# Tianion/topazdb

Measured on AMD Instinct MI355X. Metric: GiB/s device-resident SSTable block decode+checksum, 4KiB blocks, 1 MI355X, higher is better.
Workload: dtype u8; 1 GPU; 4k: 1048576 blocks/GPU x 4155 B median, 34.0 entries/block, tag 1 (Uncompress); blocks_per_gpu=1048576, input_bytes_per_gpu=4356833280, parallelism=shard1

## Files before the change

### topazdb_amd/csrc/tpz_decode.hip

```cpp

#include <hip/hip_runtime.h>
#include <stdint.h>

#include "tpz_internal.h"
#include "tpz_spill.hip"

namespace tpz {

typedef uint32_t u32;
typedef uint64_t u64;

constexpr int kWave = 64;
#ifdef TPZ_ABL_W20
#ifdef TPZ_ABL_W8
constexpr int kWavesPerWG = 8;
#else
constexpr int kWavesPerWG = 10;
#endif
#else
constexpr int kWavesPerWG = 16;
#endif
constexpr int kWGThreads = kWave * kWavesPerWG;
constexpr u32 kRowShift = 4, kRowBlocks = 1u << kRowShift;
#ifndef TPZ_ROW_AHEAD
// ... 508 lines not shown
      const uint4 v = src((int)x0 + delta);
      acc.x = (acc.x & ~byte_mask(lo, hi, 0)) | (v.x & byte_mask(lo, hi, 0));
      acc.y = (acc.y & ~byte_mask(lo, hi, 1)) | (v.y & byte_mask(lo, hi, 1));
      acc.z = (acc.z & ~byte_mask(lo, hi, 2)) | (v.z & byte_mask(lo, hi, 2));
      acc.w = (acc.w & ~byte_mask(lo, hi, 3)) | (v.w & byte_mask(lo, hi, 3));
    }
  }
  dst.put(c, acc, act);
  return carry_out;
}

template <class Col, class MapT, class S, class D>
__device__ __forceinline__ void copy_stream(const S& src, const Col& col, const MapT* map, u32 nk,
                                            u32 tot, const D& dst, u32 map_len) {
  const u32 lane = lane_id();
  const u32 nch = (tot + 15) >> 4;
  const u32 npad = (nch + 7) & ~7u;
  const u32 nw = (npad + 63) >> 6;
#ifdef TPZ_ABL_MEMONLY
  for (u32 c = lane; c < npad; c += 64) dst.put(c, make_uint4(c, 0, 0, 0), c < nch);
  return;
#endif
  u32 carry = 0;
  for (u32 w = 0; w < nw; w++) carry = copy_window(src, col, map, nk, tot, dst, map_len, w, carry);
}

struct PendingCrc {
  u32 live;
  u32 b, st, cnt, stored, k;
  u32 lc;
  u32 early;
};

__device__ __forceinline__ void finish_pending(const u32* tab, const Out& o, PendingCrc& pd) {
  if (!pd.live) return;
  const u32 R = crc_combine(tab, pd.lc);
  const u32 crc = (R == crc_shift_small(tab, ~pd.stored, pd.k)) ? pd.stored
                                                                   : ~crc_unshift_small(tab, R, pd.k);
  const bool ok = crc == pd.stored;
  put_meta(o, pd.b, ok ? pd.st : TPZ_BLOCK_CHECKSUM_MISMATCH, ok ? pd.cnt : 0u, crc);
  pd.live = 0;
}

struct FinishAtExit {
  const u32* tab;
  const Out& o;
  PendingCrc& pd;
  bool on;
  __device__ __forceinline__ ~FinishAtExit() {
    if (on) finish_pending(tab, o, pd);
  }
};

template <int J>
__device__ __forceinline__ bool comb_lane(u32 lane) {
  return J == 0 ? (lane & 1u) == 1u : J == 1 ? (lane & 3u) == 2u : J == 2 ? (lane & 7u) == 4u
       : J == 3 ? (lane & 15u) == 8u : J == 4 ? (lane & 31u) == 16u : (lane & 47u) == 32u;
}
struct CombLv {
  u32 r0, r1, r2, r3;
};
template <int J>
__device__ __forceinline__ CombLv comb_issue(const u32* tab, u32 A) {
  CombLv c;
  if (comb_lane<J>(lane_id())) {
    constexpr int b0 = 16 + 4 * J;
    c.r0 = tlook(tab, b0, A & 0xFF);
    c.r1 = tlook(tab, b0 + 1, (A >> 8) & 0xFF);
    c.r2 = tlook(tab, b0 + 2, (A >> 16) & 0xFF);
    c.r3 = tlook(tab, b0 + 3, A >> 24);
  }
  return c;
}
template <int J>
__device__ __forceinline__ u32 comb_use(u32 A, const CombLv& c) {
  if (comb_lane<J>(lane_id())) A = xor3(c.r0, c.r1, c.r2) ^ c.r3;
  if (J < 4) A ^= dpp<kRowShl + (1 << (J < 4 ? J : 0))>(A);
  return A;
}

__device__ __forceinline__ void comb_finish(const u32* tab, const Out& o, PendingCrc& pd, u32 cA,
                                            u32 want) {
  if (!pd.live) return;
  const u32 R = readlane(cA, 0) ^ readlane(cA, 16) ^ readlane(cA, 32) ^ readlane(cA, 48);
  const u32 crc = R == want ? pd.stored : ~crc_unshift_small(tab, R, pd.k);
  const bool ok = crc == pd.stored;
  put_meta(o, pd.b, ok ? pd.st : TPZ_BLOCK_CHECKSUM_MISMATCH, ok ? pd.cnt : 0u, crc);
  pd.live = 0;
}

struct CrcLane {
  int seg;
  bool act;
  u32 c;
};

__device__ __forceinline__ void crc_step(const u32* tab, const uint8_t* win, int pb, CrcLane& L,
                                         int t) {
  typedef u32 u32x4 __attribute__((ext_vector_type(4)));
  const int a = L.act ? pb + L.seg + 16 * t : -kGuard;
  const u32x4 w = *reinterpret_cast<const u32x4*>(win + a);
  L.c = slice16(tab, w.x ^ L.c, w.y, w.z, w.w);
}
__device__ __forceinline__ u32 crc_lane_value(const u32* tab, const CrcLane& L) { return L.c; }

struct FastWin {
  u32 nk, tot, nch, npad, last;
  __amdgpu_buffer_rsrc_t out;
};

template <bool FLAT, class S>
__device__ __forceinline__ u32 copy_fast(const S& src, const ColSmall& col, const uint16_t* map,
                                         const FastWin& F, const FlatOut& D, u32 w, u32 carry,
                                         u32& rare) {
  const u32 lane = lane_id();
  const u32 c = 64 * w + lane;
  const u32 x0 = 16 * c;
  const bool act = c < F.nch;
  u32 j = map[min(c, (u32)kWaveMapLen - 1)];
  j = max(wave_scan_max(act ? j : 0u), carry);
  const u32 carry_out = readlane(j, 63);
  u32 e0, e1;
  int d0, d1;
  col.get2(min(j, F.last), e0, d0, e1, d1);
  const bool cross = act && j + 1 < F.nk && e0 < x0 + 16;
  uint4 acc = src(act ? (int)x0 + d0 : -kGuard);
  const uint4 nx = src(cross ? (int)x0 + d1 : -kGuard);
  const bool rw = __ballot(act && (e0 <= x0 || (cross && e1 < x0 + 16 && j + 2 < F.nk))) != 0;
  if (rw) rare |= 1u << w;
  if (cross) acc = merge_at(acc, nx, (int)(e0 - x0));
  if (FLAT) {
    D.put(c, acc, rw);
  } else {
    __builtin_amdgcn_raw_buffer_store_b128(__builtin_bit_cast(__attribute__((ext_vector_type(4))) u32, acc),
                                           F.out, rw ? kOob : x0, 0, 0);
  }
  return carry_out;
}

template <bool FLAT, class S>
__device__ __forceinline__ u32 copy_fast3(const S& src, const ColSmall& col, const uint16_t* map,
                                          const FastWin& F, const FlatOut& D, u32 w, u32 carry,
                                          u32& rare) {
  const u32 lane = lane_id();
  const u32 c = 64 * w + lane;
  const u32 x0 = 16 * c;
  const bool act = c < F.nch;
  u32 j = map[min(c, (u32)kWaveMapLen - 1)];
  j = max(wave_scan_max(act ? j : 0u), carry);
  const u32 carry_out = readlane(j, 63);
  u32 e0, e1, e2, e3;
  int d0, d1, d2, d3;
  col.get2(min(j, F.last), e0, d0, e1, d1);
  col.get2(min(j + 2, F.last), e2, d2, e3, d3);
  if (act && e0 <= x0) {
    j++;
    e0 = e1, d0 = d1, e1 = e2, d1 = d2, e2 = e3, d2 = d3;
  }
  const bool b1 = act && j + 1 < F.nk && e0 < x0 + 16;
  const bool b2 = b1 && j + 2 < F.nk && e1 < x0 + 16;
  uint4 acc = src(act ? (int)x0 + d0 : -kGuard);
  const uint4 n1 = src(b1 ? (int)x0 + d1 : -kGuard);
  const uint4 n2 = src(b2 ? (int)x0 + d2 : -kGuard);
  const bool rw = __ballot(act && (e0 <= x0 || (b2 && e2 < x0 + 16 && j + 3 < F.nk))) != 0;
  if (rw) rare |= 1u << w;
  if (b1) acc = merge_at(acc, n1, (int)(e0 - x0));
  if (b2) acc = merge_at(acc, n2, (int)(e1 - x0));
  if (FLAT)
    D.put(c, acc, rw);
  else
    __builtin_amdgcn_raw_buffer_store_b128(__builtin_bit_cast(__attribute__((ext_vector_type(4))) u32, acc),
                                           F.out, rw ? kOob : x0, 0, 0);
  return carry_out;
}

template <bool SHORT, bool FLAT, class S>
__device__ __forceinline__ u32 copy_crc_fused(const u32* tab, const S& src, const ColSmall& col,
                                              const uint16_t* map, u32 nk, u32 tot, uint8_t* dst,
                                              const FlatOut& D, const uint8_t* win, int pb, u32 Pa,
                                              u32 kshift, Stamps& St, u32 w3, const Out& o,
                                              PendingCrc& pd) {
  const u32 lane = lane_id();
  FastWin F;
  F.nk = nk;
  F.tot = tot;
  F.nch = (tot + 15) >> 4;
  F.npad = FLAT ? F.nch : (F.nch + 7) & ~7u;
  F.last = nk ? nk - 1 : 0u;
  F.out = __builtin_amdgcn_make_buffer_rsrc(dst, (short)0, FLAT ? 0 : (int)(F.npad * 16), 0x00020000);
  const u32 nw = (F.npad + 63) >> 6;
  CrcLane L;
  L.seg = (int)Pa - kCrcLaneBytes * (int)(lane + 1);
  L.act = L.seg + kCrcLaneBytes > 0;
  L.c = 0;
  u32 carry = 0, rare = 0, cw[5];
  const bool pl = pd.live != 0;
  u32 cA = pd.lc, want = 0;
  CombLv cl{0u, 0u, 0u, 0u};
  if (pl) {
    cl = comb_issue<0>(tab, cA);
    want = crc_shift_small(tab, ~pd.stored, pd.k);
  }
#pragma unroll
  for (int t = 0; t < 4; t++) {
    cw[t] = carry;
    crc_step(tab, win, pb, L, t);
    carry = (SHORT && (u32)t < w3) ? copy_fast3<FLAT>(src, col, map, F, D, (u32)t, carry, rare)
                                   : copy_fast<FLAT>(src, col, map, F, D, (u32)t, carry, rare);
    if (pl) {
      if (t == 0) { cA = comb_use<0>(cA, cl); cl = comb_issue<1>(tab, cA); }
      if (t == 1) { cA = comb_use<1>(cA, cl); cl = comb_issue<2>(tab, cA); }
      if (t == 2) { cA = comb_use<2>(cA, cl); cl = comb_issue<3>(tab, cA); }
      if (t == 3) { cA = comb_use<3>(cA, cl); cl = comb_issue<4>(tab, cA); }
    }
  }
  cw[4] = carry;
  crc_step(tab, win, pb, L, 4);
  if (pl) {
    cA = comb_use<4>(cA, cl);
    cl = comb_issue<5>(tab, cA);
  }
  if (nw > 4)
    carry = (SHORT && 4u < w3) ? copy_fast3<FLAT>(src, col, map, F, D, 4u, carry, rare)
                               : copy_fast<FLAT>(src, col, map, F, D, 4u, carry, rare);
  if (pl) comb_finish(tab, o, pd, comb_use<5>(cA, cl), want);
  TPZ_STAMP(St, 4);
#ifdef TPZ_ABL_STAMPS
  St.rare += __builtin_popcount(rare);
#endif
  if (rare) {
    for (u32 w = 0; w < nw; w++)
      if (rare & (1u << w)) {
        if (FLAT)
          copy_window(src, col, map, nk, F.tot, FlatDst{&D}, (u32)kWaveMapLen, w, cw[w]);
        else
          copy_window(src, col, map, nk, F.tot, SlotDst{dst, F.npad, F.tot}, (u32)kWaveMapLen, w, cw[w]);
      }
  }
  return crc_lane_value(tab, L);
}

typedef u32 u32x2v __attribute__((ext_vector_type(2)));
typedef u32 u32x4v __attribute__((ext_vector_type(4)));
struct Gath {
  u32 d0, d1, d2, d3, d4;
};
__device__ __forceinline__ Gath gath_issue(const uint8_t* base, int x) {
  const u32* p = reinterpret_cast<const u32*>(base + (x & ~3));
  Gath g;
  g.d0 = p[0];
  g.d1 = p[1];
  g.d2 = p[2];
  g.d3 = p[3];
  g.d4 = p[4];
  return g;
}
__device__ __forceinline__ uint4 gath_finish(Gath g, int x) {
  asm volatile("" : "+v"(g.d0), "+v"(g.d1), "+v"(g.d2), "+v"(g.d3), "+v"(g.d4));
  const u32 s = (u32)x & 3u;
  return make_uint4(__builtin_amdgcn_alignbyte(g.d1, g.d0, s), __builtin_amdgcn_alignbyte(g.d2, g.d1, s),
                    __builtin_amdgcn_alignbyte(g.d3, g.d2, s), __builtin_amdgcn_alignbyte(g.d4, g.d3, s));
}
struct Look16 {
  u32 r[16];
};
__device__ __forceinline__ Look16 look_issue(const u32* tab, u32x4v w, u32 c) {
  Look16 L;
  const u32 w0 = w.x ^ c;
#pragma unroll
  for (int i = 0; i < 4; i++) {
    L.r[i] = tlook(tab, 15 - i, (w0 >> (8 * i)) & 0xFF);
    L.r[4 + i] = tlook(tab, 11 - i, (w.y >> (8 * i)) & 0xFF);
    L.r[8 + i] = tlook(tab, 7 - i, (w.z >> (8 * i)) & 0xFF);
    L.r[12 + i] = tlook(tab, 3 - i, (w.w >> (8 * i)) & 0xFF);
  }
  return L;
}
__device__ __forceinline__ u32 look_xor(const Look16& L) {
  u32 c = xor3(L.r[0], L.r[1], L.r[2]);
  c = xor3(c, L.r[3], L.r[4]);
  c = xor3(c, L.r[5], L.r[6]);
  c = xor3(c, L.r[7], L.r[8]);
  c = xor3(c, L.r[9], L.r[10]);
  c = xor3(c, L.r[11], L.r[12]);
  c = xor3(c, L.r[13], L.r[14]);
  return c ^ L.r[15];
}
#define TPZ_SB() __builtin_amdgcn_sched_barrier(0)

struct PWin {
  u32 m, j;
  u32 e0, e1;
  int d0, d1;
  bool act, cross;
  Gath ga, gn;
};
struct PWin3 {
  u32 e2, e3;
  int d2, d3;
  bool b2;
  Gath g2;
};

template <bool FLAT, u32 K3>
__device__ __forceinline__ u32 copy_crc_piped(const u32* tab, const ColSmall& col,
                                              const uint16_t* map, u32 nk, u32 tot, uint8_t* dst,
                                              const FlatOut& D, const uint8_t* win, int pb, u32 Pa,
                                              const Out& o, PendingCrc& pd, u32 k3n = K3) {
  const u32 lane = lane_id();
  FastWin F;
  F.nk = nk;
  F.tot = tot;
  F.nch = (tot + 15) >> 4;
  F.npad = FLAT ? F.nch : (F.nch + 7) & ~7u;
  F.last = nk ? nk - 1 : 0u;
  F.out = __builtin_amdgcn_make_buffer_rsrc(dst, (short)0, FLAT ? 0 : (int)(F.npad * 16), 0x00020000);
  const u32 nw = (F.npad + 63) >> 6;
  const int seg = (int)Pa - kCrcLaneBytes * (int)(lane + 1);
  const bool cact = seg + kCrcLaneBytes > 0;
  const int cbase = cact ? pb + seg : -kGuard;
  auto dread = [&](int t) -> u32x4v {
    return *reinterpret_cast<const u32x4v*>(win + cbase + 16 * t);
  };
  PWin W[4];
  PWin3 W3;
#pragma unroll
  for (int w = 0; w < 4; w++) {
    const u32 c = 64 * w + lane;
    W[w].act = c < F.nch;
    W[w].m = map[min(c, (u32)kWaveMapLen - 1)];
  }
  u32x4v dA = dread(0);
  u32 cA = pd.lc;
  CombLv cl = comb_issue<0>(tab, cA);
  const u32 want = crc_shift_small(tab, ~pd.stored, pd.k);
  TPZ_SB();
#pragma unroll
  for (int w = 0; w < 4; w++) W[w].j = wave_scan_max(W[w].act ? W[w].m : 0u);
  u32 cw[5];
  cw[0] = 0;
#pragma unroll
  for (int w = 0; w < 4; w++) {
    W[w].j = max(W[w].j, cw[w]);
    cw[w + 1] = readlane(W[w].j, 63);
  }
#pragma unroll
  for (int w = 0; w < 4; w++) col.get2(min(W[w].j, F.last), W[w].e0, W[w].d0, W[w].e1, W[w].d1);
  if (K3) col.get2(min(W[0].j + 2, F.last), W3.e2, W3.d2, W3.e3, W3.d3);
  cA = comb_use<0>(cA, cl);
  cl = comb_issue<1>(tab, cA);
  TPZ_SB();
  Look16 LK = look_issue(tab, dA, 0u);
  u32x4v dB = dread(1);
  cA = comb_use<1>(cA, cl);
  cl = comb_issue<2>(tab, cA);
  TPZ_SB();
  u32 rare = 0;
  auto gissue = [&](PWin& P, u32 w) {
    const u32 x0 = 16 * (64 * w + lane);
    if (w < K3 && w < k3n) {
      if (w > 0) col.get2(min(P.j + 2, F.last), W3.e2, W3.d2, W3.e3, W3.d3);
      if (P.act && P.e0 <= x0) {
        P.j++;
        P.e0 = P.e1, P.d0 = P.d1, P.e1 = W3.e2, P.d1 = W3.d2, W3.e2 = W3.e3, W3.d2 = W3.d3;
      }
      P.cross = P.act && P.j + 1 < F.nk && P.e0 < x0 + 16;
      W3.b2 = P.cross && P.j + 2 < F.nk && P.e1 < x0 + 16;
      if (__ballot(P.act && (P.e0 <= x0 || (W3.b2 && W3.e2 < x0 + 16 && P.j + 3 < F.nk))) != 0)
        rare |= 1u << w;
      W3.g2 = gath_issue(win, W3.b2 ? (int)x0 + W3.d2 : -kGuard);
    } else {
      P.cross = P.act && P.j + 1 < F.nk && P.e0 < x0 + 16;
    }
    P.ga = gath_issue(win, P.act ? (int)x0 + P.d0 : -kGuard);
    P.gn = gath_issue(win, P.cross ? (int)x0 + P.d1 : -kGuard);
  };
  auto finish = [&](PWin& P, u32 w) {
    const u32 c = 64 * w + lane;
    const u32 x0 = 16 * c;
    const bool rw = w < K3 && w < k3n && (rare & (1u << w));
    uint4 acc = gath_finish(P.ga, P.act ? (int)x0 + P.d0 : -kGuard);
    const uint4 nx = gath_finish(P.gn, P.cross ? (int)x0 + P.d1 : -kGuard);
    if (P.cross) acc = merge_at(acc, nx, (int)(P.e0 - x0));
    if (w < K3 && w < k3n) {
      const uint4 n2 = gath_finish(W3.g2, W3.b2 ? (int)x0 + W3.d2 : -kGuard);
      if (W3.b2) acc = merge_at(acc, n2, (int)(P.e1 - x0));
    }
    if (FLAT)
      D.put(c, acc, rw);
    else
      __builtin_amdgcn_raw_buffer_store_b128(__builtin_bit_cast(u32x4v, acc), F.out, rw ? kOob : x0, 0, 0);
  };
  gissue(W[0], 0);
  cA = comb_use<2>(cA, cl);
  cl = comb_issue<3>(tab, cA);
  TPZ_SB();
  u32 crc = 0;
  crc = look_xor(LK);
  LK = look_issue(tab, dB, crc);
  dA = dread(2);
  cA = comb_use<3>(cA, cl);
  cl = comb_issue<4>(tab, cA);
  TPZ_SB();
  finish(W[0], 0);
  gissue(W[1], 1);
  cA = comb_use<4>(cA, cl);
  cl = comb_issue<5>(tab, cA);
  TPZ_SB();
  crc = look_xor(LK);
  LK = look_issue(tab, dA, crc);
  dB = dread(3);
  cA = comb_use<5>(cA, cl);
  comb_finish(tab, o, pd, cA, want);
  TPZ_SB();
  finish(W[1], 1);
  gissue(W[2], 2);
  TPZ_SB();
  crc = look_xor(LK);
  LK = look_issue(tab, dB, crc);
  dA = dread(4);
  TPZ_SB();
  finish(W[2], 2);
  gissue(W[3], 3);
  TPZ_SB();
  crc = look_xor(LK);
  LK = look_issue(tab, dA, crc);
  TPZ_SB();
  finish(W[3], 3);
  TPZ_SB();
  crc = look_xor(LK);
  if (nw > 4) {
    (void)copy_fast<FLAT>(Src16{win}, col, map, F, D, 4u, cw[4], rare);
  }
  if (rare) {
    for (u32 w = 0; w < nw; w++)
      if (rare & (1u << w)) {
        if (FLAT)
          copy_window(Src16{win}, col, map, nk, F.tot, FlatDst{&D}, (u32)kWaveMapLen, w, cw[w]);
        else
          copy_window(Src16{win}, col, map, nk, F.tot, SlotDst{dst, F.npad, F.tot}, (u32)kWaveMapLen, w, cw[w]);
      }
  }
  return crc;
}


template <class Col, class MapT, int kMapLen, bool BIG, bool FLAT = false>
__device__ __forceinline__ void decode_block(const u32* tab, uint8_t* win, const Col& col,
                                             MapT* map, u32 a0, u32 len, u32 b, u64 ext_b,
                                             const Out& o, u32 kshift, Stamps& S, PendingCrc& pd,
                                             u64 kf = 0, u64 vf = 0, u64 ef = 0,
                                             const Out* o_lds = nullptr) {
  const u32 lane = lane_id();
  const u32 tag = win[(int)(a0 + len) - 1];
  const u32 stored = bswap32(lds_u32(win, len >= 5 ? a0 + len - 5 : a0));
  const u32 n = lds_be16(win, a0);
  const u32 dk = (u32)kf & 15u, dv = (u32)vf & 15u;
  u32 e_off = 0, e_kl = 0;
  bool e_ok = false;
  if (!BIG) {
    e_off = lds_be16(win, a0 + 2 + 2 * lane);
    const u32 Pn = len - 5, db0 = a0 + 2 + 2 * n;
    e_ok = len >= 7 && lane < n && Pn >= 2 + 2 * n && e_off + 2 <= Pn - 2 - 2 * n;
    e_kl = lds_be16(win, e_ok ? db0 + e_off : a0);
  }
  if (pd.early) finish_pending(tab, o, pd);
  FinishAtExit fin{tab, o, pd, true};
  if (len == 0) { put_meta(o, b, TPZ_BLOCK_EMPTY, 0, 0); return; }
  if (tag == 0 || tag > 3) { put_meta(o, b, TPZ_BLOCK_BAD_TAG, 0, 0); return; }
  if (tag != 1) { put_meta(o, b, TPZ_BLOCK_UNSUPPORTED_CODEC, 0, 0); return; }
  if (len - 1 < 4) { put_meta(o, b, TPZ_BLOCK_MALFORMED, 0, 0); return; }
  const u32 P = len - 5;
  const int pb = (int)a0;
  u32 st = TPZ_BLOCK_OK, cnt = n;
  bool fuse = false;
  bool f_short = false;
  u32 f_w3 = 0;
  u32 f_nk = 0, f_tot = 0;
  uint8_t* f_dst = nullptr;
  FlatOut fo;
  if (P < 2 || P < 2 + 2 * n) {
    st = TPZ_BLOCK_MALFORMED;
    cnt = 0;
  } else if (!BIG && n > kWaveMaxN) {
    const Out& oc = o_lds ? *o_lds : o;
    if (FLAT) defer_to(oc.spill_list, oc.spill_count, b);
    else defer_to(oc.defer_list, oc.defer_count, b);
    return;
  } else {
    const u32 db = a0 + 2 + 2 * n;
    const u32 dl = P - 2 - 2 * n;
    const bool slots_fit = FLAT || 6u * n <= len;
    uint2* ends_g = reinterpret_cast<uint2*>(o.ends) + uni64((FLAT || o.efirst) ? ef : entry_base(ext_b, b));
    const u32 n_pad = o.efirst ? n : (n + 15) & ~15u;
    {
      constexpr u32 per = 16 / sizeof(MapT);
      const u32 nz = min((u32)kMapLen, ((len >> 4) + 3 + per - 1) / per * per);
      for (u32 i = lane; i < nz / per; i += 64)
        reinterpret_cast<uint4*>(map)[i] = make_uint4(0, 0, 0, 0);
    }
    u32 ktot = 0, knz_all = 0;
    if (n > 64) {
      for (u32 g0 = 0; g0 < n; g0 += 64) {
        const u32 i = g0 + lane;
        u32 kl = 0;
        if (i < n) {
          const u32 off = lds_be16(win, a0 + 2 + 2 * i);
          if (off + 2 <= dl) {
            kl = lds_be16(win, db + off);
            if (off + 4 + kl > dl) kl = 0;
          }
        }
        knz_all += __builtin_popcountll(__ballot(kl != 0));
        ktot += readlane(wave_scan_incl(kl), 63);
      }
    }
    u32 kc = 0, vc = 0, knz = 0, vnz = 0;
    bool bad = false, short_k = false, short_v = false;
    for (u32 g0 = 0; g0 < n; g0 += 64) {
      const u32 i = g0 + lane;
      const bool act = i < n;
      u32 off = 0, kl = 0, vl = 0;
      bool ok = true;
      if (act) {
        if (!BIG && g0 == 0) {
          off = e_off;
          ok = e_ok;
          if (ok) { kl = e_kl; ok = off + 4 + kl <= dl; }
        } else {
          off = lds_be16(win, a0 + 2 + 2 * i);
          ok = off + 2 <= dl;
          if (ok) { kl = lds_be16(win, db + off); ok = off + 4 + kl <= dl; }
        }
        if (ok) { vl = lds_be16(win, db + off + 2 + kl); ok = off + 4 + kl + vl <= dl; }
        if (!ok) kl = vl = 0;
      }
      bad |= __ballot(act && !ok) != 0;
      short_k |= __ballot(kl != 0 && kl < 16) != 0;
      short_v |= __ballot(vl != 0 && vl < 16) != 0;
      const u32 ki = wave_scan_incl(kl) + kc;
      const u32 vi = wave_scan_incl(vl) + vc;
      const u64 kmask = __ballot(kl != 0), vmask = __ballot(vl != 0);
      if (n <= 64) {
        ktot = readlane(ki, 63);
        knz_all = __builtin_popcountll(kmask);
      }
      const u32 vs = stream_vstart<FLAT>(ktot, dk, dv);
      __builtin_amdgcn_raw_buffer_store_b64(
          __builtin_bit_cast(__attribute__((ext_vector_type(2))) u32,
                             act ? make_uint2(ki, vi) : make_uint2(0, 0)),
          whole_rsrc(ends_g), (slots_fit && i < n_pad) ? 8 * i : kOob, 0, 0);
      if (act && slots_fit) {
        if (kl) {
          const u32 m = knz + lanes_below(kmask);
          const u32 ke = ki + dk;
          col.put(m, ke, (int)(db + off + 2) - (int)(ke - kl));
          if (((ke + 15) >> 4) < (u32)kMapLen) map[(ke + 15) >> 4] = (MapT)(m + 1);
        }
        if (vl) {
          const u32 m = knz_all + vnz + lanes_below(vmask);
          const u32 ve = vs + vi;
          col.put(m, ve, (int)(db + off + 4 + kl) - (int)(ve - vl));
          if (((ve + 15) >> 4) < (u32)kMapLen) map[(ve + 15) >> 4] = (MapT)(m + 1);
        }
      }
      knz += __builtin_popcountll(kmask);
      vnz += __builtin_popcountll(vmask);
      kc = readlane(ki, 63);
      vc = readlane(vi, 63);
    }

    const u32 vs = stream_vstart<FLAT>(kc, dk, dv);
    TPZ_STAMP(S, 2);
    if (bad || !slots_fit || vs + vc > len + (FLAT ? 47u : 2u)) {
      const Out& oc = o_lds ? *o_lds : o;
      defer_to(oc.spill_list, oc.spill_count, b);
      return;
    } else {
      if (BIG) {
        asm volatile("s_waitcnt vmcnt(0)" ::: "memory");
        __builtin_amdgcn_fence(__ATOMIC_RELEASE, "workgroup");
      }
      __builtin_amdgcn_wave_barrier();
      const u32 tot = FLAT ? (vc ? vs + vc : (kc ? dk + kc : 0u)) : vs + vc;
#ifndef TPZ_ABL_NOCOPY
#if !defined(TPZ_ABL_NOCRC) && !defined(TPZ_ABL_MEMONLY)
#ifdef TPZ_ABL_UNFUSED
      if (false) {
#else
      if (!BIG && P >= 4) {
#endif
        fuse = true;
        f_w3 = short_v ? 5u : (short_k ? (((FLAT ? dk : 0u) + kc + 15) / 16 + 63) / 64 : 0u);
        f_short = f_w3 != 0;
        f_nk = knz + vnz;
        f_tot = tot;
        f_dst = FLAT ? nullptr : o.data + slot_base(ext_b, b);
        if (FLAT) fo = flat_out(o, kf, vf, kc, vc);
      } else
#endif
      if (FLAT) {
        fo = flat_out(o, kf, vf, kc, vc);
        copy_stream(Src16{win}, col, map, knz + vnz, tot, FlatDst{&fo}, (u32)kMapLen);
      } else {
        const u32 nch = (tot + 15) >> 4;
        copy_stream(Src16{win}, col, map, knz + vnz, tot,
                    SlotDst{o.data + slot_base(ext_b, b), (nch + 7) & ~7u, tot}, (u32)kMapLen);
      }
#endif
    }
    TPZ_STAMP(S, 3);
  }
  __builtin_amdgcn_wave_barrier();
  u32 crc;
  if (P >= 4) {
    const u32 k = ((a0 + P + 15) & ~15u) - (a0 + P);
    if (lane < 4) win[a0 + lane] ^= 0xFFu;
    if (lane < 16) win[a0 + P + lane] = 0;
    __builtin_amdgcn_wave_barrier();
#if defined(TPZ_ABL_NOCRC) || defined(TPZ_ABL_MEMONLY)
    crc = stored;
#else
    u32 R;
    if (!BIG && fuse) {
      u32 lc;
      fin.on = false;
      if (!f_short) {
        lc = copy_crc_piped<FLAT, 0u>(tab, *reinterpret_cast<const ColSmall*>(&col),
                                         reinterpret_cast<const uint16_t*>(map), f_nk, f_tot, f_dst,
                                         fo, win, pb, P + k, o, pd);
      } else if (f_w3 <= 2u) {
        lc = copy_crc_piped<FLAT, 2u>(tab, *reinterpret_cast<const ColSmall*>(&col),
                                      reinterpret_cast<const uint16_t*>(map), f_nk, f_tot, f_dst,
                                      fo, win, pb, P + k, o, pd, FLAT ? 2u : f_w3);
        f_short = false;
      } else
      {
        lc = f_short
          ? copy_crc_fused<true, FLAT>(tab, Src16{win}, *reinterpret_cast<const ColSmall*>(&col),
                                       reinterpret_cast<const uint16_t*>(map), f_nk, f_tot, f_dst,
                                       fo, win, pb, P + k, kshift, S, f_w3, o, pd)
          : copy_crc_fused<false, FLAT>(tab, Src16{win}, *reinterpret_cast<const ColSmall*>(&col),
                                        reinterpret_cast<const uint16_t*>(map), f_nk, f_tot, f_dst,
                                        fo, win, pb, P + k, kshift, S, 5u, o, pd);
      }
      pd = PendingCrc{1u, b, st, cnt, stored, k, lc, f_short ? 1u : 0u};
      return;
    } else {
        R = wave_crc(tab, win, pb, P + k);
    }
    if constexpr (BIG)
      crc = (R == crc_shift_small(tab, ~stored, k)) ? stored : ~crc_unshift_small(tab, R, k);
    else
      crc = (R == crc_shift_small(tab, ~stored, k)) ? stored : ~crc_unshift_small(tab, R, k);
#endif
  } else {
    u32 c = 0xFFFFFFFFu;
    for (u32 i = 0; i < P; i++) {
      c ^= win[a0 + i];
      for (int k = 0; k < 8; k++) c = (c >> 1) ^ (0xEDB88320u & (0u - (c & 1u)));
    }
    crc = ~c;
  }
  if (crc != stored) {
    st = TPZ_BLOCK_CHECKSUM_MISMATCH;
    cnt = 0;
  }
  TPZ_STAMP(S, 6);
  put_meta(o, b, st, cnt, crc);
}

__device__ __forceinline__ void load_tables(u32* tab, const u32* gtab, int bytes = kTableBytes) {
  const uint4* s = reinterpret_cast<const uint4*>(gtab);
  uint4* d = reinterpret_cast<uint4*>(tab);
  for (int i = threadIdx.x; i < bytes / 16; i += blockDim.x) d[i] = s[i];
  __syncthreads();
}

__device__ __forceinline__ __amdgpu_buffer_rsrc_t window_rsrc(const uint8_t* src, u64 src_bytes,
                                                               u64 wstart) {
  u64 rem = src_bytes > wstart ? src_bytes - wstart : 0;
  if (rem > 0x7FFFFFF0ull) rem = 0x7FFFFFF0ull;
  return __builtin_amdgcn_make_buffer_rsrc((void*)(src + wstart), (short)0, (int)rem, 0x00020000);
}

__device__ __forceinline__ void fix_tail(uint4& v, const uint8_t* src, u64 piece, u64 src_bytes) {
  const bool straddle = piece + 16 > src_bytes && piece < src_bytes;
  if (__ballot(straddle)) {
    u32 w[4] = {0, 0, 0, 0};
#pragma unroll
    for (u32 k = 0; k < 16; k++) {
      const u64 a = piece + k;
      const u32 byte = src[a < src_bytes ? a : src_bytes - 1];
      w[k >> 2] |= (a < src_bytes ? byte : 0u) << (8 * (k & 3));
    }
    v.x = straddle ? w[0] : v.x;
    v.y = straddle ? w[1] : v.y;
    v.z = straddle ? w[2] : v.z;
    v.w = straddle ? w[3] : v.w;
  }
}

struct Params {
  u64* big_scratch;
  u64* spill_used;
  const uint8_t* src;
  const u64* ext;
  u64 src_bytes;
  u32 n_blocks;
  const u32* crc_tables;
  Out out;
  u32 xp[kBigSuper];
  u32 lane_shift[64];
  u32 chunk_shift;
  u32* row_ctr;
  u32* err;
};


template <class T>
__device__ __forceinline__ T const_load(const T* base, u64 i) {
  return reinterpret_cast<const __attribute__((address_space(4))) T*>(reinterpret_cast<uintptr_t>(base))[i];
}

#ifdef TPZ_ABL_ROWLATE
__device__ __noinline__ void rowlate_delay(const Params& p, u32 wid, u32 point) {
  const u32 rows = (p.n_blocks + kRowBlocks - 1) / kRowBlocks;
  const u32 ctr = __hip_atomic_load(p.row_ctr, __ATOMIC_RELAXED, __HIP_MEMORY_SCOPE_AGENT);
  const bool late = point == 0 ? (wid & 1u) != 0 : (wid & 3u) == 2;
  if (late && ctr + 2 * gridDim.x >= rows)
    for (int i = 0; i < 30; i++) __builtin_amdgcn_s_sleep(127);
}
#endif
#ifdef TPZ_ABL_ONCHIP
constexpr u32 kOnchipMask = 4095;
#endif
template <bool FLAT, u32 CS>
#if defined(TPZ_ABL_W20) && !defined(TPZ_ABL_NOCAP)
__global__ __launch_bounds__(kWGThreads) __attribute__((amdgpu_waves_per_eu(5, 5)))
#else
__global__ __launch_bounds__(kWGThreads, 4)
#endif
void decode_wave_kernel(Params p) {
  __shared__ __attribute__((aligned(16))) uint8_t lds[kWaveLds];
  u32* tab = reinterpret_cast<u32*>(lds);
  __shared__ u32 chunk_next;
  __shared__ Out out_lds;
  __shared__ u64 row_ent[kRowRing];
  __shared__ u32 claims_done, exit_slot;
  if (threadIdx.x == 0) {
    claims_done = 0;
    exit_slot = ~0u;
  }
  if (threadIdx.x < kRowAhead && CS < kRowShift) {
    const u32 r0 = atomicAdd(p.row_ctr, 1u);
    row_ent[threadIdx.x] = (u64)r0 | (u64)threadIdx.x << 32;
    if ((u64)r0 * kRowBlocks >= p.n_blocks) {
      claims_done = 1;
      atomicMin(&exit_slot, kRowAhead);
    }
  } else if (threadIdx.x < kRowRing) {
    row_ent[threadIdx.x] = ~0ull;
  }
  if (threadIdx.x == 0) {
    chunk_next = 0;
    out_lds = p.out;
  }
  if (blockIdx.x == 0 && threadIdx.x == 0) *p.spill_used = 0;
  load_tables(tab, p.crc_tables, kWaveTabBytes);

  const u32 wid = uni(threadIdx.x >> 6);
  const u32 lane = lane_id();
  const u32 kshift = p.lane_shift[lane];
  uint8_t* slot = lds + kWaveTabBytes + wid * kSlotBytes;
  uint8_t* win = slot + kGuard;
  uint8_t* etab = win + kWinBytes + 32;
  const ColSmall col{reinterpret_cast<u32*>(etab)};
  uint16_t* map = reinterpret_cast<uint16_t*>(etab + kWaveTabSlots * 4);

  if (lane < kGuard / 16) reinterpret_cast<uint4*>(slot)[lane] = make_uint4(0, 0, 0, 0);
  const u32 nw = gridDim.x * kWavesPerWG;
  Stamps S;
#ifdef TPZ_ABL_STAMPS
  S.last = stamp_now();
#endif

#ifdef TPZ_WAVE_CHUNK
  const u32 cshift = __builtin_ctz((u32)TPZ_WAVE_CHUNK);
#else
  const u32 cshift = CS;
#endif
  const u32 kChunk = 1u << cshift, rshift = kRowShift - cshift;
  u32 pend_slot = ~0u, pend_row = 0;
  const u32 kq = 1u << rshift;
  auto publish = [&]() {
    if (pend_slot != ~0u) {
      if (lane == 0) {

        if ((u64)pend_row * kRowBlocks >= p.n_blocks) {
          __hip_atomic_store(&claims_done, 1u, __ATOMIC_RELAXED, __HIP_MEMORY_SCOPE_WORKGROUP);
          const u32 Q = __hip_atomic_fetch_add(&chunk_next, 0u, __ATOMIC_RELAXED,
                                               __HIP_MEMORY_SCOPE_WORKGROUP);
          atomicMin(&exit_slot, Q == 0 ? kRowAhead : (Q - 1) / kq + kRowAhead + 1);
        }
        __hip_atomic_store(&row_ent[pend_slot % kRowRing], (u64)pend_row | (u64)pend_slot << 32,
                           __ATOMIC_RELAXED, __HIP_MEMORY_SCOPE_WORKGROUP);
      }
      pend_slot = ~0u;
    }
  };
  const bool dyn_rows = rshift != 0;
  u32 q_tk = 0;
  if (lane == 0) q_tk = atomicAdd(&chunk_next, 1u);
  auto claim_chunk = [&]() -> u32 {
    for (;;) {
      publish();
      const u32 q_old = q_tk;
      if (lane == 0) q_tk = atomicAdd(&chunk_next, 1u);
      const u32 q = uni(q_old);
      if (!dyn_rows) {
        const u64 f = ((u64)q * gridDim.x + blockIdx.x) * kRowBlocks;
        return f < p.n_blocks ? (u32)f : p.n_blocks;
      }
      const u32 slot_q = q >> rshift;
      if (slot_q >= uni(__hip_atomic_load(&exit_slot, __ATOMIC_RELAXED, __HIP_MEMORY_SCOPE_WORKGROUP)))
        return p.n_blocks;
      if ((q & ((1u << rshift) - 1u)) == 0) {
#ifdef TPZ_ABL_ROWLATE
        rowlate_delay(p, wid, 0);
#endif
        if (!uni(__hip_atomic_load(&claims_done, __ATOMIC_RELAXED, __HIP_MEMORY_SCOPE_WORKGROUP))) {
          pend_slot = slot_q + kRowAhead;
#ifdef TPZ_ABL_ROWLATE
          rowlate_delay(p, wid, 1);
#endif
          if (lane == 0) pend_row = atomicAdd(p.row_ctr, 1u);
        } else if (lane == 0) {
          const u32 sx = slot_q + kRowAhead;
          __hip_atomic_store(&row_ent[sx % kRowRing], (u64)kRowExit | (u64)sx << 32, __ATOMIC_RELAXED,
                             __HIP_MEMORY_SCOPE_WORKGROUP);
        }
      }
      u32 row = 0;
      if (lane == 0) {
        u32 spins = 0;
        u64 ent;
        while ((u32)((ent = __hip_atomic_load(&row_ent[slot_q % kRowRing], __ATOMIC_RELAXED,
                                              __HIP_MEMORY_SCOPE_WORKGROUP)) >> 32) != slot_q) {
          const u32 rs = (u32)(ent >> 32);
          if (rs != ~0u && (int)(rs - slot_q) > 0) {
            atomicOr(p.err, 4u);
            break;
          }
          __builtin_amdgcn_s_sleep(2);
          if (++spins == (1u << 22)) {
            atomicOr(p.err, 2u);
            break;
          }
        }
        row = (u32)(ent >> 32) != slot_q ? kRowExit : (u32)ent;
      }
      row = uni(row);
      if (row != kRowExit) {
        const u64 f = (u64)row * kRowBlocks + ((q & ((1u << rshift) - 1u)) << cshift);
        if (f < p.n_blocks) return (u32)f;
      }
    }
  };
  auto chunk_first = [](u32 f) -> u32 { return f; };
  u64 gs_cur, gs_nxt;
  auto load_group = [&](u32 q, u64& gs) {
#ifdef TPZ_ABL_ONCHIP
    u32 bb = (chunk_first(q) & kOnchipMask) + (lane <= kChunk ? lane : 0u);
#else
    u32 bb = chunk_first(q) + (lane <= kChunk ? lane : 0u);
#endif
    bb = bb < p.n_blocks ? bb : p.n_blocks;
    gs = p.ext[bb];
  };
  auto lane64 = [](u64 x, u32 l) { return ((u64)readlane((u32)(x >> 32), l) << 32) | readlane((u32)x, l); };
  auto triage_group = [&](u32 q, u64 gs) {
    const u32 glo = (u32)__builtin_amdgcn_update_dpp((int)readlane((u32)gs, 16), (int)(u32)gs,
                                                     kRowShl + 1, 0xF, 0xF, false);
    const u32 ghi = (u32)__builtin_amdgcn_update_dpp((int)readlane((u32)(gs >> 32), 16),
                                                     (int)(u32)(gs >> 32), kRowShl + 1, 0xF, 0xF, false);
    const u64 ge = ((u64)ghi << 32) | glo;
    const u32 cf = chunk_first(q), bb = cf + lane;
    const bool lng = lane < kChunk && lane < p.n_blocks - cf && ge - gs > kWaveMaxLen;
    if (!__ballot(lng)) return;
    const Out& oc = out_lds;
    u32 nent = 0xFFFFu;
    if (lng) nent = ((u32)p.src[gs] << 8) | p.src[gs + 1];
    const bool to_bw = lng && nent < 64 && oc.bw_list && ge - gs <= TPZ_BIGWAVE_BLOCK_BYTES;
    const bool to_spill = lng && !to_bw && (FLAT || ge - gs > kBigMaxLen);
    if (oc.bw_list) defer_lanes(oc.bw_list, oc.bw_count, to_bw, (u32)bb);
    defer_lanes(oc.spill_list, oc.spill_count, to_spill, (u32)bb);
    defer_lanes(oc.defer_list, oc.defer_count, lng && !to_bw && !to_spill, (u32)bb);
  };
  u32 q_cur = claim_chunk(), q_nxt = claim_chunk();
  load_group(q_cur, gs_cur);
  load_group(q_nxt, gs_nxt);
  triage_group(q_cur, gs_cur);
  u32 j = 0;
  u32 b = chunk_first(q_cur);

  uint4 v[kWinRounds];
  u64 s_cur = 0, e_cur = 0;
  u64 kf_cur = 0, vf_cur = 0, ef_cur = 0;
  auto issue = [&](u32 bb, u32 jj, u64& s, u64& e) {
    if (FLAT && bb >= p.n_blocks) return;
    if (bb < p.n_blocks) {
      if (FLAT) {
        kf_cur = const_load(p.out.kfirst, bb);
        vf_cur = const_load(p.out.vfirst, bb);
        ef_cur = const_load(p.out.efirst, bb);
      } else if (p.out.efirst) {
        ef_cur = const_load(p.out.efirst, bb);
      }
    }
    s = lane64(gs_cur, jj);
    e = lane64(gs_cur, jj + 1);
    const bool take = bb < p.n_blocks && e - s <= kWaveMaxLen;
// ... 514 lines not shown
```

Measured before the change: 2322 GiB/s.

## Add fast path for blocks with uniform key/value lengths using closed-form indexing

After: 2410 GiB/s (median of 6 runs). +3.8%, better.

```diff
diff --git a/topazdb_amd/csrc/tpz_decode.hip b/topazdb_amd/csrc/tpz_decode.hip
--- a/topazdb_amd/csrc/tpz_decode.hip
+++ b/topazdb_amd/csrc/tpz_decode.hip
@@ -834,11 +834,28 @@
   Gath g2;
 };
 
-template <bool FLAT, u32 K3>
+struct RegGeom {
+  u32 n, KL, VL, db;
+};
+constexpr u32 kRegShift = 26;
+__device__ __forceinline__ u32 reg_recip(u32 d) {
+  u32 m = (u32)(__builtin_amdgcn_rcpf((float)d) * (float)(1u << kRegShift)) + 2u;
+  asm volatile("" : "+v"(m));
+  return uni(m);
+}
+__device__ __forceinline__ u32 mul24(u32 a, u32 b) { return (a & 0xFFFFFFu) * (b & 0xFFFFFFu); }
+__device__ __forceinline__ u32 reg_div(u32 y, u32 m) {
+  const u64 p = (u64)(y & 0x1FFFu) * (u64)(m & 0x7FFFFFu);
+  return __builtin_amdgcn_alignbit((u32)(p >> 32), (u32)p, kRegShift) & 0x3FFu;
+}
+
+template <bool FLAT, u32 K3, bool REG = false>
 __device__ __forceinline__ u32 copy_crc_piped(const u32* tab, const ColSmall& col,
                                               const uint16_t* map, u32 nk, u32 tot, uint8_t* dst,
                                               const FlatOut& D, const uint8_t* win, int pb, u32 Pa,
-                                              const Out& o, PendingCrc& pd, u32 k3n = K3) {
+                                              const Out& o, PendingCrc& pd, u32 k3n = K3,
+                                              const RegGeom G = RegGeom{0u, 0u, 0u, 0u}) {
+  static_assert(!REG || (K3 == 0 && !FLAT), "the regular copy: slotted, no short keys");
   const u32 lane = lane_id();
   FastWin F;
   F.nk = nk;
@@ -856,28 +873,52 @@
   };
   PWin W[4];
   PWin3 W3;
+  const u32 r_kc = G.n * G.KL, r_vs = (r_kc + 15) & ~15u, r_S = 4 + G.KL + G.VL;
+  const u32 r_mk = REG ? reg_recip(G.KL) : 0u, r_mv = REG ? reg_recip(G.VL) : 0u;
+  const int r_gap = (int)(2 + G.KL) - (int)r_vs - (int)((G.n - 1) * (4 + G.VL));
+  auto reg_entry = [&](PWin& P, u32 x0, bool isk) {
+    const u32 L = isk ? G.KL : G.VL, base = isk ? 0u : r_vs, T = r_S - L;
+    const u32 j = reg_div(x0 - base, isk ? r_mk : r_mv);
+    const bool last = j + 1 == G.n;
+    P.j = 0;
+    P.e0 = (!isk && last) ? 0xFFFFu : base + mul24(j + 1, L);
+    P.d0 = (int)((isk ? G.db + 2 : G.db + 4 + G.KL - r_vs) + mul24(j, T));
+    P.d1 = P.d0 + ((isk && last) ? r_gap : (int)T);
+  };
+  auto reg_index = [&](PWin& P, u32 w) {
+    const u32 x0 = 16 * (64 * w + lane);
+    if (1024 * (w + 1) <= r_kc) reg_entry(P, x0, true);
+    else if (1024 * w >= r_vs) reg_entry(P, x0, false);
+    else reg_entry(P, x0, x0 < r_kc);
+    asm volatile("" : "+v"(P.e0), "+v"(P.d0), "+v"(P.d1));
+  };
 #pragma unroll
   for (int w = 0; w < 4; w++) {
     const u32 c = 64 * w + lane;
     W[w].act = c < F.nch;
-    W[w].m = map[min(c, (u32)kWaveMapLen - 1)];
+    if (!REG) W[w].m = map[min(c, (u32)kWaveMapLen - 1)];
   }
   u32x4v dA = dread(0);
   u32 cA = pd.lc;
   CombLv cl = comb_issue<0>(tab, cA);
   const u32 want = crc_shift_small(tab, ~pd.stored, pd.k);
   TPZ_SB();
-#pragma unroll
-  for (int w = 0; w < 4; w++) W[w].j = wave_scan_max(W[w].act ? W[w].m : 0u);
   u32 cw[5];
   cw[0] = 0;
+  if (REG) {
 #pragma unroll
-  for (int w = 0; w < 4; w++) {
-    W[w].j = max(W[w].j, cw[w]);
-    cw[w + 1] = readlane(W[w].j, 63);
-  }
+    for (int w = 0; w < 4; w++) reg_index(W[w], (u32)w);
+  } else {
 #pragma unroll
-  for (int w = 0; w < 4; w++) col.get2(min(W[w].j, F.last), W[w].e0, W[w].d0, W[w].e1, W[w].d1);
+    for (int w = 0; w < 4; w++) W[w].j = wave_scan_max(W[w].act ? W[w].m : 0u);
+#pragma unroll
+    for (int w = 0; w < 4; w++) {
+      W[w].j = max(W[w].j, cw[w]);
+      cw[w + 1] = readlane(W[w].j, 63);
+    }
+#pragma unroll
+    for (int w = 0; w < 4; w++) col.get2(min(W[w].j, F.last), W[w].e0, W[w].d0, W[w].e1, W[w].d1);
+  }
   if (K3) col.get2(min(W[0].j + 2, F.last), W3.e2, W3.d2, W3.e3, W3.d3);
   cA = comb_use<0>(cA, cl);
   cl = comb_issue<1>(tab, cA);
@@ -962,9 +1003,16 @@
   TPZ_SB();
   crc = look_xor(LK);
   if (nw > 4) {
-    (void)copy_fast<FLAT>(Src16{win}, col, map, F, D, 4u, cw[4], rare);
-  }
-  if (rare) {
+    if (REG) {
+      W[0].act = 256 + lane < F.nch;
+      reg_index(W[0], 4u);
+      gissue(W[0], 4u);
+      finish(W[0], 4u);
+    } else {
+      (void)copy_fast<FLAT>(Src16{win}, col, map, F, D, 4u, cw[4], rare);
+    }
+  }
+  if (!REG && rare) {
     for (u32 w = 0; w < nw; w++)
       if (rare & (1u << w)) {
         if (FLAT)
@@ -976,6 +1024,15 @@
   return crc;
 }
 
+
+__device__ __forceinline__ u32 crc_prepare(uint8_t* win, u32 a0, u32 P) {
+  const u32 lane = lane_id();
+  const u32 k = ((a0 + P + 15) & ~15u) - (a0 + P);
+  if (lane < 4) win[a0 + lane] ^= 0xFFu;
+  if (lane < 16) win[a0 + P + lane] = 0;
+  __builtin_amdgcn_wave_barrier();
+  return k;
+}
 
 template <class Col, class MapT, int kMapLen, bool BIG, bool FLAT = false>
 __device__ __forceinline__ void decode_block(const u32* tab, uint8_t* win, const Col& col,
@@ -1025,6 +1082,46 @@
     const bool slots_fit = FLAT || 6u * n <= len;
     uint2* ends_g = reinterpret_cast<uint2*>(o.ends) + uni64((FLAT || o.efirst) ? ef : entry_base(ext_b, b));
     const u32 n_pad = o.efirst ? n : (n + 15) & ~15u;
+    u32 r_vl = 0;
+    bool r_ok = false;
+    if constexpr (!BIG && !FLAT) {
+      r_ok = e_ok && e_off + 4 + e_kl <= dl;
+      if (r_ok) { r_vl = lds_be16(win, db + e_off + 2 + e_kl); r_ok = e_off + 4 + e_kl + r_vl <= dl; }
+      const u32 KL = readlane(e_kl, 0), VL = readlane(r_vl, 0), es = 4 + KL + VL;
+      bool reg = n != 0 && KL >= 16 && VL >= 16 && P >= 4 && slots_fit &&
+                 !__ballot(lane < n && !(r_ok && e_off == mul24(lane, es) && e_kl == KL && r_vl == VL));
+      for (u32 g0 = 64; reg && g0 < n; g0 += 64) {
+        const u32 i = g0 + lane;
+        bool same = true;
+        if (i < n) {
+          const u32 off = lds_be16(win, a0 + 2 + 2 * i);
+          same = off == mul24(i, es) && off + 4 + KL + VL <= dl;
+          if (same) same = lds_be16(win, db + off) == KL && lds_be16(win, db + off + 2 + KL) == VL;
+        }
+        reg = !__ballot(!same);
+      }
+      const u32 kc = n * KL, vc = n * VL, vs = stream_vstart<false>(kc, 0u, 0u);
+      if (reg && vs + vc <= len + 2u) {
+        for (u32 g0 = 0; g0 < n; g0 += 64) {
+          const u32 i = g0 + lane;
+          __builtin_amdgcn_raw_buffer_store_b64(
+              __builtin_bit_cast(__attribute__((ext_vector_type(2))) u32,
+                                 i < n ? make_uint2(mul24(i + 1, KL), mul24(i + 1, VL)) : make_uint2(0, 0)),
+              whole_rsrc(ends_g), i < n_pad ? 8 * i : kOob, 0, 0);
+        }
+        TPZ_STAMP(S, 2);
+        TPZ_STAMP(S, 3);
+        __builtin_amdgcn_wave_barrier();
+        const u32 k = crc_prepare(win, a0, P);
+        fin.on = false;
+        const u32 lc = copy_crc_piped<false, 0u, true>(
+            tab, *reinterpret_cast<const ColSmall*>(&col), reinterpret_cast<const uint16_t*>(map),
+            2 * n, vs + vc, o.data + slot_base(ext_b, b), fo, win, pb, P + k, o, pd, 0u,
+            RegGeom{n, KL, VL, db});
+        pd = PendingCrc{1u, b, st, cnt, stored, k, lc, 0u};
+        return;
+      }
+    }
     {
       constexpr u32 per = 16 / sizeof(MapT);
       const u32 nz = min((u32)kMapLen, ((len >> 4) + 3 + per - 1) / per * per);
@@ -1055,16 +1152,23 @@
       u32 off = 0, kl = 0, vl = 0;
       bool ok = true;
       if (act) {
-        if (!BIG && g0 == 0) {
+        if (!BIG && !FLAT && g0 == 0) {
           off = e_off;
-          ok = e_ok;
-          if (ok) { kl = e_kl; ok = off + 4 + kl <= dl; }
+          kl = e_kl;
+          vl = r_vl;
+          ok = r_ok;
         } else {
-          off = lds_be16(win, a0 + 2 + 2 * i);
-          ok = off + 2 <= dl;
-          if (ok) { kl = lds_be16(win, db + off); ok = off + 4 + kl <= dl; }
+          if (!BIG && g0 == 0) {
+            off = e_off;
+            ok = e_ok;
+            if (ok) { kl = e_kl; ok = off + 4 + kl <= dl; }
+          } else {
+            off = lds_be16(win, a0 + 2 + 2 * i);
+            ok = off + 2 <= dl;
+            if (ok) { kl = lds_be16(win, db + off); ok = off + 4 + kl <= dl; }
+          }
+          if (ok) { vl = lds_be16(win, db + off + 2 + kl); ok = off + 4 + kl + vl <= dl; }
         }
-        if (ok) { vl = lds_be16(win, db + off + 2 + kl); ok = off + 4 + kl + vl <= dl; }
         if (!ok) kl = vl = 0;
       }
       bad |= __ballot(act && !ok) != 0;
@@ -1146,10 +1250,7 @@
   __builtin_amdgcn_wave_barrier();
   u32 crc;
   if (P >= 4) {
-    const u32 k = ((a0 + P + 15) & ~15u) - (a0 + P);
-    if (lane < 4) win[a0 + lane] ^= 0xFFu;
-    if (lane < 16) win[a0 + P + lane] = 0;
-    __builtin_amdgcn_wave_barrier();
+    const u32 k = crc_prepare(win, a0, P);
 #if defined(TPZ_ABL_NOCRC) || defined(TPZ_ABL_MEMONLY)
     crc = stored;
 #else
```
